# penn-graphics-research/claymore

Measured on AMD Instinct MI355X. Metric: particles*steps/sec, higher is better.
Workload: dtype f32

## Files before the change

claymore_amd/csrc/claymore_hip.hip:

```cpp
#include <hip/hip_runtime.h>

#include <algorithm>
#include <cmath>
#include <cstdio>
#include <cstdlib>
#include <chrono>
#include <cstring>
#include <string>
#include <vector>

#include "../../include/claymore_amd.h"
#include "mpm_kernels.hpp"
#include "mpm_readout.hpp"

using namespace mpm;
#define MPM_STR_(x) #x
#define MPM_STR(x) MPM_STR_(x)

namespace {
constexpr int kHaloWords	 = 128;
constexpr int kStatusBlock = ST_WORDS + kHaloWords + kMaxVelSlots * kMaxVelStride;

struct Partition {
	int* table = nullptr;
// ... 99 lines not shown
		}
	}
};

#define HIP_TRY(expr)                                                                                            \
	do {                                                                                                         \
		hipError_t e_ = (expr);                                                                                  \
		if(e_ != hipSuccess) {                                                                                   \
			ctx->err = std::string(#expr) + " -> " + hipGetErrorString(e_) + " (" + __FILE__ + ":" + std::to_string(__LINE__) + ")"; \
			return MPM_ERR_DEVICE;                                                                               \
		}                                                                                                        \
	} while(0)

static float host_maxvel(const mpm_ctx* ctx) {
	float m = 0.f;
	for(int i = 0; i < kMaxVelSlots; ++i) m = std::max(m, ctx->h_maxvel[i * kMaxVelStride]);
	return m;
}

#ifndef MPM_PAIR_BUILD
#define MPM_PAIR_BUILD 0xF
#endif
#ifndef MPM_PAIR_DEFAULT
#define MPM_PAIR_DEFAULT 0xF
#endif
static int pair_mask() {
	static const int mask = [] {
		const char* e = std::getenv("MPM_G2P2G_PAIRS");
		return (e && *e ? (int) std::strtol(e, nullptr, 0) : MPM_PAIR_DEFAULT) & MPM_PAIR_BUILD;
	}();
	return mask;
}

static int launch_prepare(mpm_ctx* ctx, int cur, int prev, bool list_is_out, int binoff_sel, const int* pbc_ptr, int nblocks_est, bool sort, bool publish);

static int fail(mpm_ctx* ctx, int code, const std::string& msg) {
	ctx->err = msg;
	return code;
}

static inline void phase_call(mpm_ctx* ctx) {
	if(ctx) ctx->group_summed = false;
}

template<typename T>
static hipError_t dalloc(T** p, size_t n) {
	return hipMalloc((void**) p, sizeof(T) * (n ? n : 1));
}

template<typename T>
struct DevScratch {
	T* p = nullptr;
	DevScratch() = default;
	DevScratch(const DevScratch&) = delete;
	DevScratch& operator=(const DevScratch&) = delete;
	~DevScratch() {
		if(p) hipFree(p);
	}
	hipError_t alloc(size_t n) { return dalloc(&p, n); }
};

template<typename T>
static hipError_t regrow(T** p, size_t old_n, size_t new_n, hipStream_t s) {
	T* q		 = nullptr;
	hipError_t e = hipMalloc((void**) &q, sizeof(T) * new_n);
	if(e != hipSuccess) return e;
	if((e = hipMemsetAsync(q, 0, sizeof(T) * new_n, s)) != hipSuccess || (*p && old_n && (e = hipMemcpyAsync(q, *p, sizeof(T) * old_n, hipMemcpyDeviceToDevice, s)) != hipSuccess)
// ... 246 lines not shown
	HIP_TRY(hipMemsetAsync(ctx->d_status, 0, sizeof(int) * kStatusBlock, s));
	for(int i = 0; i < 2; ++i) {
		HIP_TRY(dalloc(&ctx->part[i].table, table));
		HIP_TRY(dalloc(&ctx->part[i].count, 1));
		HIP_TRY(hipMemsetAsync(ctx->part[i].table, 0xff, sizeof(int) * table, s));
		HIP_TRY(hipMemsetAsync(ctx->part[i].count, 0, sizeof(int), s));
	}
	size_t total_particles = 0;
	for(auto& m: ctx->models) total_particles += m.n;
	size_t prov = std::min(table, total_particles + 1);
	if(ctx->cfg.max_blocks > 0) prov = std::min<size_t>(table, (size_t) ctx->cfg.max_blocks);
	Partition& P = ctx->part[n];
	HIP_TRY(dalloc(&P.keys, 3 * prov));
	g.cap = (int) prov;
	for(auto& m: ctx->models)
		if(m.n) activate_blocks_kernel<<<cdiv(m.n, 256), 256, 0, s>>>(g, m.n, m.d_xyz, P.table, P.keys, P.count, ctx->d_status);
	int pbc = 0;
	HIP_TRY(hipMemcpyAsync(&pbc, P.count, sizeof(int), hipMemcpyDeviceToHost, s));
	HIP_TRY(hipStreamSynchronize(s));
	if(pbc > g.cap) return fail(ctx, MPM_ERR_CAPACITY, "Too much active blocks: " + std::to_string(pbc));
	ctx->pbc = pbc;
	if(ctx->cfg.max_blocks <= 0 && (size_t) pbc * 27 > prov) {
		int* keys		  = nullptr;
		const size_t need = std::min(table, (size_t) pbc * 27 + 1);
		HIP_TRY(dalloc(&keys, 3 * need));
		HIP_TRY(hipMemcpyAsync(keys, P.keys, sizeof(int) * 3 * (size_t) pbc, hipMemcpyDeviceToDevice, s));
		HIP_TRY(hipStreamSynchronize(s));
		HIP_TRY(hipFree(P.keys));
		P.keys = keys;
		prov   = need;
		g.cap  = (int) prov;
	}
	HIP_TRY(hipMemcpyAsync(&ctx->d_status[ST_CNT_P], P.count, sizeof(int), hipMemcpyDeviceToDevice, s));
	register_blocks_kernel<0, 1><<<std::max(1u, std::min(4096u, cdiv((size_t) pbc * 8, 256))), 256, 0, s>>>(g, &ctx->d_status[ST_CNT_P], nullptr, &ctx->d_status[ST_CNT_N], &ctx->d_status[ST_PBC], P.table, P.keys, ctx->d_status);
	register_blocks_kernel<-1, 1><<<std::max(1u, std::min(8192u, cdiv((size_t) pbc * 32, 256))), 256, 0, s>>>(g, &ctx->d_status[ST_CNT_P], &ctx->d_status[ST_CNT_N], &ctx->d_status[ST_CNT_E], &ctx->d_status[ST_NBC], P.table, P.keys, ctx->d_status);
	{
		int rc0 = read_status(ctx);
		if(rc0) return rc0;
		rc0 = check_status(ctx);
		if(rc0) return rc0;
		const int ebc0 = ctx->h_status[ST_CNT_P] + ctx->h_status[ST_CNT_N] + ctx->h_status[ST_CNT_E];
		ctx->h_status[ST_EBC] = ebc0;
		ctx->pbc_prev		  = pbc;
		HIP_TRY(hipMemcpyAsync(&ctx->d_status[ST_EBC], &ctx->h_status[ST_EBC], sizeof(int), hipMemcpyHostToDevice, s));
		HIP_TRY(hipMemcpyAsync(&ctx->d_status[ST_PBCPREV], &ctx->pbc_prev, sizeof(int), hipMemcpyHostToDevice, s));
		HIP_TRY(hipMemcpyAsync(P.count, &ctx->h_status[ST_EBC], sizeof(int), hipMemcpyHostToDevice, s));
		HIP_TRY(hipStreamSynchronize(s));
	}
	ctx->nbc = ctx->h_status[ST_NBC];
	ctx->ebc = ctx->h_status[ST_EBC];
	size_t cap = ctx->cfg.max_blocks > 0 ? (size_t) ctx->cfg.max_blocks : std::min(table, (size_t) ctx->ebc * 3 / 2 + 4096);
	if(cap < (size_t) ctx->ebc) return fail(ctx, MPM_ERR_CAPACITY, "Too much exterior blocks: " + std::to_string(ctx->ebc) + " (max_blocks " + std::to_string(cap) + ")");
	{
		int* keys = nullptr;
		HIP_TRY(dalloc(&keys, 3 * cap));
		HIP_TRY(hipMemcpyAsync(keys, P.keys, sizeof(int) * 3 * (size_t) ctx->ebc, hipMemcpyDeviceToDevice, s));
		HIP_TRY(hipStreamSynchronize(s));
		HIP_TRY(hipFree(P.keys));
		P.keys = keys;
		HIP_TRY(dalloc(&ctx->part[r].keys, 3 * cap));
	}
	g.cap = (int) cap;
	for(int i = 0; i < 2; ++i) {
		HIP_TRY(dalloc(&ctx->grid[i], cap * 256));
	}
	for(size_t mi = 0; mi < ctx->models.size(); ++mi) {
		Model& m  = ctx->models[mi];
		m.bin_cap = m.n / kBin + cap + 1;
// ... 197 lines not shown
		for(auto& m: ctx->models) launch_g2p2g_model(ctx, m, nullptr, &ctx->d_status[ST_PBC], ctx->pbc, dt, next_dt, s);
	HIP_TRY(hipEventRecord(e1, s));
	return MPM_OK;
}

int mpm_g2p2g(mpm_ctx* ctx, float dt, float next_dt) {
	phase_call(ctx);
	if(!ctx || !ctx->ready) return MPM_ERR_NOT_READY;
	HIP_TRY(hipSetDevice(ctx->device));
	int rc = launch_g2p2g(ctx, dt, next_dt, ctx->ev.g2p2g_start, ctx->ev.g2p2g_end);
	if(rc) return rc;
	HIP_TRY(hipGetLastError());
	HIP_TRY(hipStreamSynchronize(ctx->s_compute));
	HIP_TRY(hipEventElapsedTime(&ctx->last_g2p2g_ms, ctx->ev.g2p2g_start, ctx->ev.g2p2g_end));
	ctx->timers.g2p2g_ms = ctx->last_g2p2g_ms;
	return MPM_OK;
}

static int launch_prepare(mpm_ctx* ctx, int cur, int prev, bool list_is_out, int binoff_sel, const int* pbc_ptr, int nblocks_est, bool sort, bool publish) {
	if(nblocks_est <= 0 && !publish) return MPM_OK;
	PrepareModels pm {};
	pm.n = (int) ctx->models.size();
	for(int mi = 0; mi < pm.n; ++mi) {
		Model& m		  = ctx->models[mi];
		pm.list[mi]		  = m.list[list_is_out ? (m.list_in ^ 1) : m.list_in];
		pm.size[mi]		  = m.size;
		pm.row_of[mi]	  = m.row_of;
		pm.binoff_src[mi] = m.binoff[binoff_sel];
		pm.blockinfo[mi]  = m.blockinfo;
		pm.keep[mi]		  = sort && list_is_out ? m.keep : nullptr;
		pm.pairinfo[mi]	  = m.pair ? m.pairinfo[0] : nullptr;
		pm.pairhand[mi]	  = m.pairinfo[1];
	}
	const int nwg = std::max(1, std::min(ctx->g.cap, nblocks_est + nblocks_est / 16 + 64));
	int* pub	  = publish ? ctx->d_status : nullptr;
	if(sort)
		prepare_blocks_kernel<true><<<nwg, 64, 0, ctx->s_compute>>>(ctx->g, pm, pbc_ptr, ctx->part[cur].table, ctx->part[cur].keys, ctx->part[prev].table, pub, ctx->part[cur].count);
	else
		prepare_blocks_kernel<false><<<nwg, 64, 0, ctx->s_compute>>>(ctx->g, pm, pbc_ptr, ctx->part[cur].table, ctx->part[cur].keys, ctx->part[prev].table, pub, ctx->part[cur].count);
	return MPM_OK;
}

static int launch_rebuild_prepare(mpm_ctx* ctx) {
	const int r = ctx->rollid, n = r ^ 1;
	const int ebc_est = std::min(ctx->g.cap, ctx->ebc + ctx->ebc / 16 + 1024);
	return launch_prepare(ctx, n, r, true, n, &ctx->d_status[ST_CNT_P], ebc_est, true, true);
}
static int launch_rebuild(mpm_ctx* ctx, float fuse_dt = 0.f, bool without_prepare = false) {
	if(fuse_dt == 0.f) fuse_dt = ctx->fuse_dt_once;
	ctx->fuse_dt_once = 0.f;
	hipStream_t s = ctx->s_compute;
	GridCfg& g	  = ctx->g;
	const int r = ctx->rollid, n = r ^ 1;
	Partition& Pn = ctx->part[n];
	Partition& Pr = ctx->part[r];
	const bool fused = fuse_dt > 0.f;
	ctx->grid_momentum = !fused;
	int rc			 = launch_clear(ctx, kClearRebuild | (fused ? kClearMaxVel : 0));
	if(rc) return rc;
	RebuildModels rm {};
	rm.n = (int) ctx->models.size();
	for(int mi = 0; mi < rm.n; ++mi) {
		Model& m		 = ctx->models[mi];
		rm.out_count[mi] = m.out_count;
		rm.size[mi]		 = m.size;
		rm.row_of[mi]	 = m.row_of;
		rm.binoff[mi]	 = m.binoff[r];
		rm.bin_cap[mi]	 = (long long) m.bin_cap;
	}
	int* st			  = ctx->d_status;
	const int ebc_est = std::min(g.cap, ctx->ebc + ctx->ebc / 16 + 1024);
	compact_blocks_kernel<<<std::max(1u, cdiv(ebc_est, 1024)), 1024, 0, s>>>(g, rm, Pr.keys, Pn.keys, Pn.table, st);
	const unsigned rg8 = std::max(1u, std::min(4096u, cdiv((size_t) ebc_est * 8, 256))), rg32 = std::max(1u, std::min(8192u, cdiv((size_t) ebc_est * 32, 256)));
	register_blocks_kernel<0, 1><<<rg8, 256, 0, s>>>(g, &st[ST_CNT_P], nullptr, &st[ST_CNT_N], &st[ST_PBC], Pn.table, Pn.keys, st);
	if(fused) {
		if(ctx->has_collision)
			carry_grid_kernel<true, true><<<2048, 256, 0, s>>>(g, st, Pn.keys, Pr.table, ctx->grid[1], ctx->grid[0], fuse_dt, ctx->d_maxvel, collision_tick(ctx, fuse_dt));
		else
			carry_grid_kernel<true><<<2048, 256, 0, s>>>(g, st, Pn.keys, Pr.table, ctx->grid[1], ctx->grid[0], fuse_dt, ctx->d_maxvel, NoCollision {});
		ctx->grid_preupdated = true;
		ctx->preupdate_dt	 = fuse_dt;
	} else
		carry_grid_kernel<false><<<2048, 256, 0, s>>>(g, st, Pn.keys, Pr.table, ctx->grid[1], ctx->grid[0], 0.f, nullptr, NoCollision {});
	register_blocks_kernel<-1, 1><<<rg32, 256, 0, s>>>(g, &st[ST_CNT_P], &st[ST_CNT_N], &st[ST_CNT_E], &st[ST_NBC], Pn.table, Pn.keys, st);
	if(without_prepare) return MPM_OK;
	return launch_prepare(ctx, n, r, true, n, &st[ST_CNT_P], ebc_est, true, true);
}

static int grow_capacity(mpm_ctx* ctx) {
	if(!ctx->cfg.grow) return MPM_OK;
	hipStream_t s	   = ctx->s_compute;
	const size_t table = (size_t) ctx->g.G * ctx->g.G * ctx->g.G;
	const size_t cap   = (size_t) ctx->g.cap;
	if((size_t) ctx->ebc * 4 > cap * 3 && cap < table) {
		const size_t ncap = std::min(table, cap * 3 / 2 + 1);
		HIP_TRY(hipDeviceSynchronize());
		for(int i = 0; i < 2; ++i) {
			HIP_TRY(regrow(&ctx->part[i].keys, 3 * cap, 3 * ncap, s));
			HIP_TRY(regrow(&ctx->grid[i], cap * 256, ncap * 256, s));
		}
		for(auto& m: ctx->models) {
			for(int i = 0; i < 2; ++i) {
				HIP_TRY(regrow(&m.binoff[i], cap + 1, ncap + 1, s));
				HIP_TRY(regrow(&m.list[i], cap * (size_t) ctx->g.ppb, ncap * (size_t) ctx->g.ppb, s));
			}
			HIP_TRY(regrow(&m.size, cap + 1, ncap + 1, s));
			HIP_TRY(regrow(&m.row_of, cap + 1, ncap + 1, s));
			HIP_TRY(regrow(&m.out_count, cap + 1, ncap + 1, s));
			HIP_TRY(regrow(&m.keep, cap + 1, ncap + 1, s));
			HIP_TRY(regrow(&m.blockinfo, cap * (size_t) kInfoRow, ncap * (size_t) kInfoRow, s));
			if(m.pair)
				for(int i = 0; i < 2; ++i) HIP_TRY(regrow(&m.pairinfo[i], (cap + 1) * (size_t) kPairChunks, (ncap + 1) * (size_t) kPairChunks, s));
		}
		if(ctx->d_overlap) {
			HIP_TRY(regrow(&ctx->d_overlap, cap + 1, ncap + 1, s));
			HIP_TRY(regrow(&ctx->d_halo_list, cap + 1, ncap + 1, s));
			HIP_TRY(regrow(&ctx->d_inner_list, cap + 1, ncap + 1, s));
// ... 524 lines not shown
```

claymore_amd/csrc/mpm_g2p2g.hpp:

```cpp
#pragma once
#include "mpm_device_math.hpp"

namespace mpm {

#if !(defined(MPM_EXPERIMENT) && defined(MPM_G2P2G_WAVES_FLUID))
#define MPM_G2P2G_WAVES_FLUID 4
#endif
#if !(defined(MPM_EXPERIMENT) && defined(MPM_G2P2G_WAVES))
#define MPM_G2P2G_WAVES 3
#endif

constexpr int kP2GStrideX = 36, kP2GStrideY = 6, kP2GNodes = 216;
constexpr int kP2GArena2 = 228;
constexpr int kG2PStrideX = 6, kG2PStrideY = 1, kG2PStrideZ = 36, kG2PNodes = 216;

struct ModelView {
	const float* bins_src;
	float* bins_dst;
	const int* binoff_src;
	const int* binoff_dst;
	const int* list_in;
	int* list_out;
	const int* size;
	const int* row_of;
// ... 364 lines not shown
	float am;
	StressScale ss;
	float jdiv, jvisc;
	float refl_lim;
};

MPM_DEV int code_key(int c) {
	return ((c >> 4) & 15) * 36 + (c & 15) * 6 + (c >> 8);
}
MPM_DEV bool code_edge(int c) {
	const int x = c & 15, y = (c >> 4) & 15, z = c >> 8;
	return (x == 0) | (x == 5) | (y == 0) | (y == 5) | (z == 0) | (z == 5);
}
MPM_DEV int code_off(int c) {
	return ((c & 15) - 1) * kP2GStrideX + (((c >> 4) & 15) - 1) * kP2GStrideY + ((c >> 8) - 1);
}

template<int MAT>
__global__ __launch_bounds__(kG2P2GThreads, MAT == 0 ? MPM_G2P2G_WAVES_FLUID : MPM_G2P2G_WAVES) void g2p2g_kernel(GridCfg cfg, ModelView mv, const int* __restrict__ cur_keys, const float* __restrict__ grid, float* __restrict__ next_grid, const int* __restrict__ block_list, const int* __restrict__ only_flag, const int* __restrict__ nblocks_ptr, int nblocks, float dt, float new_dt, StepConst sk, int* __restrict__ status) {
	constexpr int NCH = MatTraits<MAT>::nch;
	constexpr int REC = MatTraits<MAT>::rec;
	__shared__ float4 g2p[kG2PNodes];
	__shared__ float4 p2g[kP2GArena2 + kP2GNodes];
	__shared__ unsigned char s_owner[2 * 216];
	constexpr bool kQueue = MAT != 0 && kSerialQueue > 0;
	__shared__ float4 s_queue[kQueue ? 4 * kSerialQueue : 1];
#if defined(MPM_EXPERIMENT) && defined(MPM_LDS_PAD)
	__shared__ float s_pad[MPM_LDS_PAD / 4];
	if(size_t(grid) == 1) s_pad[threadIdx.x] = 0.f;
#endif

	const int lane0 = threadIdx.x;
	const int total = nblocks_ptr ? min(*nblocks_ptr, cfg.cap) : nblocks;
	const int xcd = (int) (blockIdx.x & 7u), nq = nblocks_ptr ? (int) (gridDim.x >> 3) : 0x40000000;
	const int share = (total >> 3) + (xcd < (total & 7) ? 1 : 0);
	const int first = xcd * (total >> 3) + min(xcd, total & 7);
	for(int q = (int) (blockIdx.x >> 3); q < share; q += nq) {
	int lane = lane0;
	__asm__ volatile("" : "+v"(lane));
	const int bid = first + q;
	const int b	  = block_list ? block_list[bid] : bid;
	const int size		 = mv.size[b];
	const int row		 = mv.row_of[b];
	const int binoff_dst = mv.binoff_dst[b];
	const int flag = only_flag ? only_flag[b] : 1;
	if(size == 0 || flag == 0) continue;
	const int* list		= mv.list_in + (size_t) row * cfg.ppb;
	const float mass	= mv.mc.mass;
	const int key_shift = cfg.pid_bits;
	const int tag_shift = cfg.pid_bits + kKeyBits;
	const int info = mv.blockinfo[(size_t) b * kInfoRow + lane];
	int cnt_cur	   = slice_records_at(size, 0);
	int cnt_next   = 64 < size ? slice_records_at(size, 64) : 1;
	int rec_cur	   = list[min(lane, cnt_cur - 1)];
	int rec_next   = list[(64 < size ? 64 : 0) + min(lane, cnt_next - 1)];
	for(int i = lane; i < kP2GArena2 + kP2GNodes; i += 64) p2g[i] = make_float4(0.f, 0.f, 0.f, 0.f);
	__syncthreads();
	float4 gv[8];
#pragma unroll
	for(int lb = 0; lb < 8; ++lb) {
		const int nb	= __shfl(info, 54 + lb);
		const float* gb = grid + (size_t) (nb < 0 ? 0 : nb) * 256;
		gv[lb].x		= gb[64 + lane];
		gv[lb].y		= gb[128 + lane];
		gv[lb].z		= gb[192 + lane];
		if(nb < 0) gv[lb].x = gv[lb].y = gv[lb].z = 0.f;
		gv[lb].w = gv[lb].z;
	}
	constexpr int ROW = NCH - REC;
// ... 321 lines not shown
```

claymore_amd/csrc/mpm_g2p2g_pair.hpp:

```cpp
#pragma once
#include "mpm_g2p2g.hpp"

namespace mpm {

#if !(defined(MPM_EXPERIMENT) && defined(MPM_PAIR_WAVES))
#define MPM_PAIR_WAVES 3
#endif
#if !(defined(MPM_EXPERIMENT) && defined(MPM_PAIR_WAVES_FLUID))
#define MPM_PAIR_WAVES_FLUID 4
#endif
#if !(defined(MPM_EXPERIMENT) && defined(MPM_PAIR_DUAL))
#define MPM_PAIR_DUAL 0
#endif
#if !(defined(MPM_EXPERIMENT) && defined(MPM_PAIR_LATE_FETCH_FLUID))
#define MPM_PAIR_LATE_FETCH_FLUID 1
#endif
#if !(defined(MPM_EXPERIMENT) && defined(MPM_PAIR_LATE_FETCH_NACC))
#define MPM_PAIR_LATE_FETCH_NACC 1
#endif
#if !(defined(MPM_EXPERIMENT) && defined(MPM_PAIR_LATE_FETCH))
#define MPM_PAIR_LATE_FETCH 0
#endif
#if !(defined(MPM_EXPERIMENT) && defined(MPM_PAIR_SHARED_GATHER))
#define MPM_PAIR_SHARED_GATHER 0x0
// ... 244 lines not shown
		const int i = o / 9, j = (o / 3) % 3, k = o % 3;
		node0[i * kP2GStrideX + j * kP2GStrideY + k] = make_float4(a01.x, a01.y, a23.x, a23.y);
		__asm__ volatile("" ::: "memory");
		if(o + 1 < 27) {
			const int i1 = (o + 1) / 9, j1 = ((o + 1) / 3) % 3, k1 = (o + 1) % 3;
			acc			 = node0[i1 * kP2GStrideX + j1 * kP2GStrideY + k1];
		}
	}
	template<int SITE>
	MPM_DEV void at() {
		static_assert(SITE >= 0 && SITE < NSITES, "site out of range");
		if(win) {
#pragma unroll
			for(int o = SITE * 27 / NSITES; o < (SITE + 1) * 27 / NSITES; ++o) step(o);
		}
	}
#endif
};

template<int MAT>
__global__ __launch_bounds__(kG2P2GThreads, MAT == 0 ? MPM_PAIR_WAVES_FLUID : MPM_PAIR_WAVES) void g2p2g_pair_kernel(GridCfg cfg, ModelView mv, const int* __restrict__ cur_keys, const float* __restrict__ grid, float* __restrict__ next_grid, const int* __restrict__ block_list, const int* __restrict__ only_flag, const int* __restrict__ nblocks_ptr, int nblocks, float dt, float new_dt, StepConst sk, int* __restrict__ status) {
	constexpr int NCH = MatTraits<MAT>::nch;
	constexpr int REC = MatTraits<MAT>::rec;
	constexpr bool kSharedGather = ((MPM_PAIR_SHARED_GATHER >> MAT) & 1) != 0;
	constexpr int kLateFetch	 = MAT == 0 ? MPM_PAIR_LATE_FETCH_FLUID : (MAT == 3 ? MPM_PAIR_LATE_FETCH_NACC : MPM_PAIR_LATE_FETCH);
	__shared__ float4 g2p[kG2PNodes];
	__shared__ float4 p2g[kP2GArena2 + kP2GNodes];
	__shared__ unsigned char s_owner[2 * 216];
	constexpr bool kQueue = MAT != 0 && kSerialQueue > 0;
	__shared__ float4 s_queue[kQueue ? 4 * kSerialQueue : 1];

	const int lane0 = threadIdx.x;
	const int total = nblocks_ptr ? min(*nblocks_ptr, cfg.cap) : nblocks;
	const int xcd = (int) (blockIdx.x & 7u), nq = nblocks_ptr ? (int) (gridDim.x >> 3) : 0x40000000;
	const int share = (total >> 3) + (xcd < (total & 7) ? 1 : 0);
	const int first = xcd * (total >> 3) + min(xcd, total & 7);
	for(int q = (int) (blockIdx.x >> 3); q < share; q += nq) {
	int lane = lane0;
	__asm__ volatile("" : "+v"(lane));
	const int bid = first + q;
	const int b	  = block_list ? block_list[bid] : bid;
	const int size		 = mv.size[b];
	const int row		 = mv.row_of[b];
	const int binoff_dst = mv.binoff_dst[b];
	const int flag		 = only_flag ? only_flag[b] : 1;
	if(size == 0 || flag == 0) continue;
	const int* list		= mv.list_in + (size_t) row * cfg.ppb;
	const float mass	= mv.mc.mass;
	const int key_shift = cfg.pid_bits;
	const int tag_shift = cfg.pid_bits + kKeyBits;
	const int info		= mv.blockinfo[(size_t) b * kInfoRow + lane];
	int chunk_nrec;
	{
		const int nch = pair_chunks(size), cl = lane & (kPairChunks - 1);
		chunk_nrec	  = cl < nch ? (cl + 1 < nch ? 512 : size - 512 * cl) : 0;
	}
	const int pinfo		= (mv.pairinfo_in[(size_t) b * kPairChunks + (lane & (kPairChunks - 1))] & 0xffff) | (chunk_nrec << 16);
	int d_slice = 0;
	auto form_slices = [&](int first) {
		int before = 0;
		d_slice = 0;
#pragma unroll 1
		for(int c = 0; c < kPairChunks; ++c) {
			const int pe = __builtin_amdgcn_readlane(pinfo, c);
			if((pe >> 16) == 0) break;
			const PairChunk pc = pair_chunk(pe >> 16, pe & 0xffff);
			const int t		   = first + lane - before;
			if(t >= 0 && t < pc.S) {
				int pos, ca, cb;
// ... 404 lines not shown
```

claymore_amd/csrc/mpm_kernels.hpp:

```cpp
#pragma once
#include <hip/hip_runtime.h>
#include <type_traits>

#include "mpm_device_math.hpp"
#include "mpm_collision.hpp"

namespace mpm {

constexpr int kBin		  = 64;
constexpr int kG2P2GThreads = 64;
constexpr int kMaxModels  = 8;
constexpr int kSortKeys		= 216;
constexpr int kKeyBits		= 8;
constexpr int kStay		  = 13;

enum {
	ST_PBC = 0, ST_NBC = 1, ST_EBC = 2, ST_OVERFLOW = 3, ST_LOST = 4, ST_ARENA = 5, ST_DROPPED = 6, ST_NONFINITE = 7, ST_BINS0 = 8, ST_PART0 = 16,
	 ST_CNT_P = 29, ST_CNT_N = 30, ST_CNT_E = 31, ST_BINSPREV = 32, ST_PBCPREV = 40, ST_WORDS = 64
};

struct GridCfg {
	int G;
	int gbits;
	int ppb;
	int pid_bits;
	int boundary;
	int cap;
	float dx, dx_inv, d_inv, gravity;
};

__device__ __forceinline__ bool key_ok(const GridCfg& c, int x, int y, int z) {
	return ((unsigned) x < (unsigned) c.G) & ((unsigned) y < (unsigned) c.G) & ((unsigned) z < (unsigned) c.G);
}
__device__ __forceinline__ size_t key_index(const GridCfg& c, int x, int y, int z) {
	return ((size_t) x << (2 * c.gbits)) | ((size_t) y << c.gbits) | (size_t) z;
}
__device__ __forceinline__ int table_query(const GridCfg& c, const int* __restrict__ table, int x, int y, int z) {
	return key_ok(c, x, y, z) ? table[key_index(c, x, y, z)] : -1;
}
__device__ __forceinline__ void table_insert(const GridCfg& c, int* table, int* keys, int* count, int x, int y, int z, int* status) {
	if(!key_ok(c, x, y, z)) return;
	const size_t i = key_index(c, x, y, z);
	if(table[i] != -1) return;
	if(atomicCAS(&table[i], -1, -2) == -1) {
		const int idx = atomicAdd(count, 1);
		if(idx < c.cap) {
			table[i]		 = idx;
			keys[3 * idx]	 = x;
			keys[3 * idx + 1] = y;
			keys[3 * idx + 2] = z;
		} else {
			table[i] = -1;
			atomicOr(&status[ST_OVERFLOW], 1);
		}
	}
}

__device__ __forceinline__ int wave_append(int* counter, bool pred) {
	const unsigned long long m = __ballot(pred);
	if(m == 0ull) return -1;
	const int lane	 = threadIdx.x & 63;
	const int leader = __ffsll((long long) m) - 1;
	int base		 = 0;
	if(lane == leader) base = atomicAdd(counter, __popcll(m));
	base = __shfl(base, leader);
	return pred ? base + __popcll(m & ((1ull << lane) - 1ull)) : -1;
}


__device__ __forceinline__ int wave_scan_incl(int v) {
	v += __builtin_amdgcn_update_dpp(0, v, 0x111, 0xf, 0xf, false);
// ... 226 lines not shown
	if(i < n) out[i] = make_float4(sd[i], gx[i], gy[i], gz[i]);
}

__device__ __forceinline__ void dir_components(int dir, int& dx, int& dy, int& dz) {
	dz = (dir % 3) - 1;
	dy = ((dir / 3) % 3) - 1;
	dx = (dir / 9) - 1;
}

constexpr int kInfoRow = 64;
struct PrepareModels {
	int n;
	int* list[kMaxModels];
	const int* size[kMaxModels];
	const int* row_of[kMaxModels];
	const int* binoff_src[kMaxModels];
	int* blockinfo[kMaxModels];
	const int* keep[kMaxModels];
	int* pairinfo[kMaxModels];
	const int* pairhand[kMaxModels];
};
template<bool SORT>
__global__ __launch_bounds__(64) void prepare_blocks_kernel(GridCfg cfg, PrepareModels pm, const int* __restrict__ pbc_ptr, const int* __restrict__ cur_table, const int* __restrict__ cur_keys, const int* __restrict__ prev_table, int* __restrict__ publish, int* __restrict__ part_count) {
	constexpr int kPrepChunk = kListChunk;
	__shared__ int s_sorted[kPairChunkMax];
	__shared__ int s_cnt[256];
	__shared__ int s_cur[256];
	const int lane = threadIdx.x;
	if(publish && blockIdx.x == 0 && lane == 0) {
		const int ebc	 = publish[ST_CNT_P] + publish[ST_CNT_N] + publish[ST_CNT_E];
		publish[ST_EBC] = ebc;
		*part_count		 = ebc;
	}
	const int pbc = min(*pbc_ptr, cfg.cap);
	for(int b = blockIdx.x; b < pbc; b += gridDim.x) {
	const int kx = cur_keys[3 * b], ky = cur_keys[3 * b + 1], kz = cur_keys[3 * b + 2];
	int size0 = 0, row0 = 0, keep0 = -2, hand0 = 0;
	if constexpr(SORT) {
		if(pm.n > 0) {
			size0 = pm.size[0][b];
			row0  = pm.row_of[0][b];
			if(pm.keep[0]) keep0 = pm.keep[0][row0];
			if(pm.pairinfo[0]) hand0 = pm.pairhand[0][(size_t) row0 * kPairChunks + (lane & (kPairChunks - 1))];
		}
	}
	int srcno = -1, other = -1;
	if(lane < 27) {
		int ox, oy, oz;
		dir_components(lane, ox, oy, oz);
		srcno = table_query(cfg, prev_table, kx + ox, ky + oy, kz + oz);
	} else if(lane < 54) {
		int ox, oy, oz;
		dir_components(lane - 27, ox, oy, oz);
		other = table_query(cfg, cur_table, kx - ox, ky - oy, kz - oz);
	} else if(lane < 62) {
		const int lb = lane - 54;
		other		 = table_query(cfg, cur_table, kx + ((lb >> 2) & 1), ky + ((lb >> 1) & 1), kz + (lb & 1));
	}
	const int key_shift		= cfg.pid_bits;
	const int tag_shift		= cfg.pid_bits + kKeyBits;
	const unsigned rec_mask = (1u << (tag_shift + 5)) - 1u;
	for(int m = 0; m < pm.n; ++m) {
		int info = other;
		if constexpr(SORT) {
		const int size = __builtin_amdgcn_readfirstlane(m == 0 ? size0 : pm.size[m][b]);
		const int row  = __builtin_amdgcn_readfirstlane(m == 0 ? row0 : pm.row_of[m][b]);
		int* list	   = pm.list[m] + (size_t) row * cfg.ppb;
		const int tail	= size & (kPrepChunk - 1);
// ... 203 lines not shown
enum { kClearP2G = 1, kClearRebuild = 2, kClearMaxVel = 4 };
struct ClearArgs {
	int flags;
	int nmodels;
	int* out_count[kMaxModels];
	int* keep[kMaxModels];
	float* p2g_grid;
	int* status;
	unsigned* max_vel_bits;
	int* old_table;
	const int* old_keys;
	const int* old_count;
};
__global__ __launch_bounds__(256) void substep_clear_kernel(GridCfg cfg, ClearArgs a) {
	const int tid = blockIdx.x * 256 + threadIdx.x, nthreads = gridDim.x * 256;
	if(a.flags & kClearP2G) {
		const int nbc = min(a.status[ST_NBC], cfg.cap), ebc = min(a.status[ST_EBC], cfg.cap);
		float4* g	  = reinterpret_cast<float4*>(a.p2g_grid);
		for(int i = tid; i < nbc * 64; i += nthreads) g[i] = make_float4(0.f, 0.f, 0.f, 0.f);
		for(int m = 0; m < a.nmodels; ++m)
			for(int i = tid; i <= ebc; i += nthreads) a.out_count[m][i] = 0, a.keep[m][i] = -1;
	}
	if(a.flags & kClearRebuild) {
		const int n = min(*a.old_count, cfg.cap);
		for(int i = tid; i < n; i += nthreads) a.old_table[key_index(cfg, a.old_keys[3 * i], a.old_keys[3 * i + 1], a.old_keys[3 * i + 2])] = -1;
		if(blockIdx.x == gridDim.x - 1) {
			if(threadIdx.x < kMaxModels) {
				a.status[ST_BINSPREV + threadIdx.x] = a.status[ST_BINS0 + threadIdx.x];
				a.status[ST_BINS0 + threadIdx.x]	= 0;
				a.status[ST_PART0 + threadIdx.x]	= 0;
			}
			if(threadIdx.x >= 8 && threadIdx.x < 11) a.status[ST_CNT_P + threadIdx.x - 8] = 0;
			if(threadIdx.x == 11) a.status[ST_PBCPREV] = a.status[ST_PBC];
			if(threadIdx.x >= 64 && threadIdx.x < 64 + kMaxVelSlots) {
				unsigned* slot = a.max_vel_bits + (threadIdx.x - 64) * kMaxVelStride;
				if(*slot >= 0x7f800000u) a.status[ST_NONFINITE] = 1;
				if(a.flags & kClearMaxVel) *slot = 0u;
			}
		}
	}
}

__global__ __launch_bounds__(1024) void compact_blocks_kernel(GridCfg cfg, RebuildModels rm, const int* __restrict__ old_keys, int* __restrict__ new_keys, int* __restrict__ new_table, int* __restrict__ status) {
	__shared__ int s_part[kMaxModels];
	const int ebc = min(status[ST_EBC], cfg.cap);
	for(int b0 = blockIdx.x * blockDim.x; b0 < ebc; b0 += gridDim.x * blockDim.x) {
		const int b = b0 + threadIdx.x;
		int c[kMaxModels];
		bool any = false;
		for(int m = 0; m < rm.n; ++m) {
			c[m] = b < ebc ? rm.out_count[m][b] : 0;
			if(c[m] > cfg.ppb) {
				atomicAdd(&status[ST_DROPPED], c[m] - cfg.ppb);
				c[m] = cfg.ppb;
			}
			any |= c[m] > 0;
		}
		__syncthreads();
		if(threadIdx.x < kMaxModels) s_part[threadIdx.x] = 0;
		__syncthreads();
		for(int m = 0; m < rm.n; ++m) {
			int t = c[m];
#pragma unroll
			for(int off = 32; off > 0; off >>= 1) t += __shfl_xor(t, off);
			if((threadIdx.x & 63) == 0 && t) atomicAdd(&s_part[m], t);
		}
		__syncthreads();
		if((int) threadIdx.x < rm.n && s_part[threadIdx.x]) atomicAdd(&status[ST_PART0 + threadIdx.x], s_part[threadIdx.x]);
		const int nb = block_append(&status[ST_CNT_P], any ? 1 : 0);
		int kx = 0, ky = 0, kz = 0;
		if(any) {
			kx = old_keys[3 * b], ky = old_keys[3 * b + 1], kz = old_keys[3 * b + 2];
			new_keys[3 * nb]					  = kx;
			new_keys[3 * nb + 1]				  = ky;
			new_keys[3 * nb + 2]				  = kz;
			new_table[key_index(cfg, kx, ky, kz)] = nb;
		}
		for(int m = 0; m < rm.n; ++m) {
			const int nbins = any ? (c[m] + kBin - 1) / kBin : 0;
			const int first = block_append(&status[ST_BINS0 + m], nbins);
			if(any) {
				const bool fits = (long long) first + nbins <= rm.bin_cap[m];
				if(!fits) atomicOr(&status[ST_OVERFLOW], 4);
				rm.size[m][nb]	 = fits ? c[m] : 0;
				rm.row_of[m][nb] = b;
				rm.binoff[m][nb] = (nbins && fits) ? first : 0;
			}
		}
	}
}

template<int LO, int HI>
__global__ __launch_bounds__(256) void register_blocks_kernel(GridCfg cfg, const int* __restrict__ pbc_ptr, const int* __restrict__ base2_ptr, int* counter, int* publish, int* table, int* keys, int* status) {
	constexpr int W	   = HI - LO + 1;
	constexpr int NOFF = W * W * W;
	constexpr int LPB  = NOFF <= 8 ? 8 : 32;
	const int pbc	   = min(*pbc_ptr, cfg.cap);
	const int base	   = *pbc_ptr + (base2_ptr ? *base2_ptr : 0);
	if(publish && blockIdx.x == 0 && threadIdx.x == 0) *publish = base;
	const long long total = (long long) pbc * LPB;
	const long long bound = (total + blockDim.x - 1) / blockDim.x * blockDim.x;
	for(long long t = (long long) blockIdx.x * blockDim.x + threadIdx.x; t < bound; t += (long long) gridDim.x * blockDim.x) {
		const int b = (int) (t / LPB), o = (int) (t % LPB);
		bool claim	= false;
		int x = 0, y = 0, z = 0;
		size_t i = 0;
		if(t < total && o < NOFF) {
			x = keys[3 * b] + LO + o / (W * W);
			y = keys[3 * b + 1] + LO + (o / W) % W;
			z = keys[3 * b + 2] + LO + o % W;
			if(key_ok(cfg, x, y, z)) {
				i = key_index(cfg, x, y, z);
				if(table[i] == -1) claim = atomicCAS(&table[i], -1, -2) == -1;
			}
		}
		const int idx = base + block_append(counter, claim ? 1 : 0);
		if(claim) {
			if(idx < cfg.cap) {
				table[i]		  = idx;
				keys[3 * idx]	  = x;
				keys[3 * idx + 1] = y;
				keys[3 * idx + 2] = z;
			} else {
				table[i] = -1;
				atomicOr(&status[ST_OVERFLOW], 1);
			}
		}
	}
}

template<bool UPDATE, bool COLLIDE = false>
__global__ __launch_bounds__(256) void carry_grid_kernel(GridCfg cfg, const int* __restrict__ status, const int* __restrict__ new_keys, const int* __restrict__ old_table, const float* __restrict__ p2g_grid, float* __restrict__ grid, float dt, unsigned* __restrict__ max_vel_bits, std::conditional_t<COLLIDE, CollisionArgs, NoCollision> col) {
	static_assert(UPDATE || !COLLIDE, "the collision object belongs to the grid update");
	const int nbc	  = min(status[ST_CNT_P] + status[ST_CNT_N], cfg.cap);
	const int old_nbc = min(status[ST_NBC], cfg.cap);
	const int lane = threadIdx.x & 63;
	float vel_sqr  = 0.f;
	for(int nb = blockIdx.x * 4 + (threadIdx.x >> 6); nb < nbc; nb += gridDim.x * 4) {
		const int kx = new_keys[3 * nb], ky = new_keys[3 * nb + 1], kz = new_keys[3 * nb + 2];
		const int old = table_query(cfg, old_table, kx, ky, kz);
		float4 v	  = {0.f, 0.f, 0.f, 0.f};
		if(old >= 0 && old < old_nbc) {
			const float* s = p2g_grid + (size_t) old * 256;
			v			   = {s[lane], s[64 + lane], s[128 + lane], s[192 + lane]};
		}
		if constexpr(COLLIDE) {
			if(v.x > 0.0f) vel_sqr = fmaxf(vel_sqr, grid_cell_collision(cfg, col, kx, ky, kz, lane, dt, v));
		} else if constexpr(UPDATE) {
			if(v.x > 0.0f) {
				const bool wx = kx < cfg.boundary || kx >= cfg.G - cfg.boundary;
				const bool wy = ky < cfg.boundary || ky >= cfg.G - cfg.boundary;
				const bool wz = kz < cfg.boundary || kz >= cfg.G - cfg.boundary;
				const float mass_inv = 1.f / v.x;
				const float v0		 = wx ? 0.0f : v.y * mass_inv;
				const float v1		 = (wy ? 0.0f : v.z * mass_inv) + cfg.gravity * dt;
				const float v2		 = wz ? 0.0f : v.w * mass_inv;
				v.y					 = v0;
				v.z					 = v1;
				v.w					 = v2;
				float q				 = v0 * v0 + v1 * v1 + v2 * v2;
				if(q != q) q = __builtin_inff();
				vel_sqr = fmaxf(vel_sqr, q);
			}
		}
		float* d	  = grid + (size_t) nb * 256;
		d[lane]		  = v.x;
		d[64 + lane]  = v.y;
		d[128 + lane] = v.z;
		d[192 + lane] = v.w;
	}
	if constexpr(UPDATE) {
#pragma unroll
		for(int off = 32; off > 0; off >>= 1) vel_sqr = fmaxf(vel_sqr, __shfl_xor(vel_sqr, off));
		if(lane == 0 && vel_sqr > 0.f) {
			const unsigned bits = __float_as_uint(vel_sqr);
			unsigned* slot		= max_vel_bits + (blockIdx.x & (kMaxVelSlots - 1)) * kMaxVelStride;
			if(bits > __hip_atomic_load(slot, __ATOMIC_RELAXED, __HIP_MEMORY_SCOPE_AGENT)) atomicMax(slot, bits);
		}
	}
}

__device__ __forceinline__ void particle_block_key(const GridCfg& cfg, const float* xyz, size_t i, int& bx, int& by, int& bz, int& cellx, int& celly, int& cellz) {
	cellx = node_index(xyz[3 * i], cfg.dx_inv) - 2;
	celly = node_index(xyz[3 * i + 1], cfg.dx_inv) - 2;
	cellz = node_index(xyz[3 * i + 2], cfg.dx_inv) - 2;
	bx	  = cellx / 4;
	by	  = celly / 4;
	bz	  = cellz / 4;
}
__global__ void activate_blocks_kernel(GridCfg cfg, size_t n, const float* __restrict__ xyz, int* table, int* keys, int* count, int* status) {
	const size_t i = (size_t) blockIdx.x * blockDim.x + threadIdx.x;
	if(i >= n) return;
	int bx, by, bz, cx, cy, cz;
	particle_block_key(cfg, xyz, i, bx, by, bz, cx, cy, cz);
	table_insert(cfg, table, keys, count, bx, by, bz, status);
}
__global__ void bucket_particles_kernel(GridCfg cfg, size_t n, const float* __restrict__ xyz, const int* __restrict__ table, int* counts, int* ids, int* status) {
	const size_t i = (size_t) blockIdx.x * blockDim.x + threadIdx.x;
	if(i >= n) return;
	int bx, by, bz, cx, cy, cz;
	particle_block_key(cfg, xyz, i, bx, by, bz, cx, cy, cz);
	const int bno = table_query(cfg, table, bx, by, bz);
	if(bno < 0) {
		atomicAdd(&status[ST_LOST], 1);
		return;
	}
	const int slot = atomicAdd(&counts[bno], 1);
	if(slot >= cfg.ppb) {
		atomicOr(&status[ST_OVERFLOW], 2);
		return;
	}
	ids[(size_t) bno * cfg.ppb + slot] = (int) i;
// ... 133 lines not shown
```

Baseline: 34.39 billion.

## Fuse grid carry with exterior block registration and partition work per XCD

In the fused rebuild path, the carry_grid kernel and the exterior register_blocks kernel are merged into one launch. Workgroups split by role: every third group per XCD registers blocks and the rest carry grid data. Registration, prepare and carry loops now hand each XCD a contiguous range of blocks, and launch sizes are rounded up to a multiple of 8. Carry reads the previous NBC from a new snapshot slot because registration now runs concurrently and overwrites ST_NBC. The aim is to save a kernel launch and serialization and to improve L2 locality per XCD, at the cost of a fixed role ratio that may load-balance poorly.

```diff
diff --git a/claymore_amd/csrc/claymore_hip.hip b/claymore_amd/csrc/claymore_hip.hip
--- a/claymore_amd/csrc/claymore_hip.hip
+++ b/claymore_amd/csrc/claymore_hip.hip
@@ -155,7 +155,18 @@
 	return mask;
 }
 
+static bool carry_split() {
+	static const bool split = [] {
+		const char* e = std::getenv("MPM_CARRY_SPLIT");
+		return e && e[0] == '1';
+	}();
+	return split;
+}
+
 static int launch_prepare(mpm_ctx* ctx, int cur, int prev, bool list_is_out, int binoff_sel, const int* pbc_ptr, int nblocks_est, bool sort, bool publish);
+static inline unsigned xcd_launch(size_t nwg) {
+	return (unsigned) ((std::max<size_t>(nwg, 1) + 7) & ~(size_t) 7);
+}
 
 static int fail(mpm_ctx* ctx, int code, const std::string& msg) {
 	ctx->err = msg;
@@ -468,8 +479,8 @@
 		g.cap  = (int) prov;
 	}
 	HIP_TRY(hipMemcpyAsync(&ctx->d_status[ST_CNT_P], P.count, sizeof(int), hipMemcpyDeviceToDevice, s));
-	register_blocks_kernel<0, 1><<<std::max(1u, std::min(4096u, cdiv((size_t) pbc * 8, 256))), 256, 0, s>>>(g, &ctx->d_status[ST_CNT_P], nullptr, &ctx->d_status[ST_CNT_N], &ctx->d_status[ST_PBC], P.table, P.keys, ctx->d_status);
-	register_blocks_kernel<-1, 1><<<std::max(1u, std::min(8192u, cdiv((size_t) pbc * 32, 256))), 256, 0, s>>>(g, &ctx->d_status[ST_CNT_P], &ctx->d_status[ST_CNT_N], &ctx->d_status[ST_CNT_E], &ctx->d_status[ST_NBC], P.table, P.keys, ctx->d_status);
+	register_blocks_kernel<0, 1><<<xcd_launch(std::min(4096u, cdiv((size_t) pbc * 8, 256))), 256, 0, s>>>(g, &ctx->d_status[ST_CNT_P], nullptr, &ctx->d_status[ST_CNT_N], &ctx->d_status[ST_PBC], P.table, P.keys, ctx->d_status);
+	register_blocks_kernel<-1, 1><<<xcd_launch(std::min(8192u, cdiv((size_t) pbc * 32, 256))), 256, 0, s>>>(g, &ctx->d_status[ST_CNT_P], &ctx->d_status[ST_CNT_N], &ctx->d_status[ST_CNT_E], &ctx->d_status[ST_NBC], P.table, P.keys, ctx->d_status);
 	{
 		int rc0 = read_status(ctx);
 		if(rc0) return rc0;
@@ -733,7 +744,7 @@
 		pm.pairinfo[mi]	  = m.pair ? m.pairinfo[0] : nullptr;
 		pm.pairhand[mi]	  = m.pairinfo[1];
 	}
-	const int nwg = std::max(1, std::min(ctx->g.cap, nblocks_est + nblocks_est / 16 + 64));
+	const unsigned nwg = xcd_launch((size_t) std::max(1, std::min(ctx->g.cap, nblocks_est + nblocks_est / 16 + 64)));
 	int* pub	  = publish ? ctx->d_status : nullptr;
 	if(sort)
 		prepare_blocks_kernel<true><<<nwg, 64, 0, ctx->s_compute>>>(ctx->g, pm, pbc_ptr, ctx->part[cur].table, ctx->part[cur].keys, ctx->part[prev].table, pub, ctx->part[cur].count);
@@ -772,18 +783,26 @@
 	int* st			  = ctx->d_status;
 	const int ebc_est = std::min(g.cap, ctx->ebc + ctx->ebc / 16 + 1024);
 	compact_blocks_kernel<<<std::max(1u, cdiv(ebc_est, 1024)), 1024, 0, s>>>(g, rm, Pr.keys, Pn.keys, Pn.table, st);
-	const unsigned rg8 = std::max(1u, std::min(4096u, cdiv((size_t) ebc_est * 8, 256))), rg32 = std::max(1u, std::min(8192u, cdiv((size_t) ebc_est * 32, 256)));
+	const unsigned rg8 = xcd_launch(std::min(4096u, cdiv((size_t) ebc_est * 8, 256))), rg32 = xcd_launch(std::min(8192u, cdiv((size_t) ebc_est * 32, 256)));
 	register_blocks_kernel<0, 1><<<rg8, 256, 0, s>>>(g, &st[ST_CNT_P], nullptr, &st[ST_CNT_N], &st[ST_PBC], Pn.table, Pn.keys, st);
 	if(fused) {
-		if(ctx->has_collision)
-			carry_grid_kernel<true, true><<<2048, 256, 0, s>>>(g, st, Pn.keys, Pr.table, ctx->grid[1], ctx->grid[0], fuse_dt, ctx->d_maxvel, collision_tick(ctx, fuse_dt));
+		const bool split = carry_split();
+		if(ctx->has_collision) {
+			if(split)
+				carry_grid_kernel<true, true><<<2048, 256, 0, s>>>(g, st, Pn.keys, Pr.table, ctx->grid[1], ctx->grid[0], fuse_dt, ctx->d_maxvel, collision_tick(ctx, fuse_dt));
+			else
+				carry_register_kernel<true, true><<<kCarryRegisterGrid, 256, 0, s>>>(g, st, Pn.keys, Pn.table, Pr.table, ctx->grid[1], ctx->grid[0], fuse_dt, ctx->d_maxvel, collision_tick(ctx, fuse_dt));
+		} else if(split)
+			carry_grid_kernel<true><<<2048, 256, 0, s>>>(g, st, Pn.keys, Pr.table, ctx->grid[1], ctx->grid[0], fuse_dt, ctx->d_maxvel, NoCollision {});
 		else
-			carry_grid_kernel<true><<<2048, 256, 0, s>>>(g, st, Pn.keys, Pr.table, ctx->grid[1], ctx->grid[0], fuse_dt, ctx->d_maxvel, NoCollision {});
+			carry_register_kernel<true><<<kCarryRegisterGrid, 256, 0, s>>>(g, st, Pn.keys, Pn.table, Pr.table, ctx->grid[1], ctx->grid[0], fuse_dt, ctx->d_maxvel, NoCollision {});
+		if(split) register_blocks_kernel<-1, 1><<<rg32, 256, 0, s>>>(g, &st[ST_CNT_P], &st[ST_CNT_N], &st[ST_CNT_E], &st[ST_NBC], Pn.table, Pn.keys, st);
 		ctx->grid_preupdated = true;
 		ctx->preupdate_dt	 = fuse_dt;
-	} else
+	} else {
 		carry_grid_kernel<false><<<2048, 256, 0, s>>>(g, st, Pn.keys, Pr.table, ctx->grid[1], ctx->grid[0], 0.f, nullptr, NoCollision {});
-	register_blocks_kernel<-1, 1><<<rg32, 256, 0, s>>>(g, &st[ST_CNT_P], &st[ST_CNT_N], &st[ST_CNT_E], &st[ST_NBC], Pn.table, Pn.keys, st);
+		register_blocks_kernel<-1, 1><<<rg32, 256, 0, s>>>(g, &st[ST_CNT_P], &st[ST_CNT_N], &st[ST_CNT_E], &st[ST_NBC], Pn.table, Pn.keys, st);
+	}
 	if(without_prepare) return MPM_OK;
 	return launch_prepare(ctx, n, r, true, n, &st[ST_CNT_P], ebc_est, true, true);
 }
diff --git a/claymore_amd/csrc/mpm_g2p2g.hpp b/claymore_amd/csrc/mpm_g2p2g.hpp
--- a/claymore_amd/csrc/mpm_g2p2g.hpp
+++ b/claymore_amd/csrc/mpm_g2p2g.hpp
@@ -420,9 +420,8 @@
 
 	const int lane0 = threadIdx.x;
 	const int total = nblocks_ptr ? min(*nblocks_ptr, cfg.cap) : nblocks;
-	const int xcd = (int) (blockIdx.x & 7u), nq = nblocks_ptr ? (int) (gridDim.x >> 3) : 0x40000000;
-	const int share = (total >> 3) + (xcd < (total & 7) ? 1 : 0);
-	const int first = xcd * (total >> 3) + min(xcd, total & 7);
+	const XcdShare xs = xcd_share(total, nblocks_ptr != nullptr);
+	const int nq = xs.nq, share = xs.share, first = xs.first;
 	for(int q = (int) (blockIdx.x >> 3); q < share; q += nq) {
 	int lane = lane0;
 	__asm__ volatile("" : "+v"(lane));
diff --git a/claymore_amd/csrc/mpm_g2p2g_pair.hpp b/claymore_amd/csrc/mpm_g2p2g_pair.hpp
--- a/claymore_amd/csrc/mpm_g2p2g_pair.hpp
+++ b/claymore_amd/csrc/mpm_g2p2g_pair.hpp
@@ -300,9 +300,8 @@
 
 	const int lane0 = threadIdx.x;
 	const int total = nblocks_ptr ? min(*nblocks_ptr, cfg.cap) : nblocks;
-	const int xcd = (int) (blockIdx.x & 7u), nq = nblocks_ptr ? (int) (gridDim.x >> 3) : 0x40000000;
-	const int share = (total >> 3) + (xcd < (total & 7) ? 1 : 0);
-	const int first = xcd * (total >> 3) + min(xcd, total & 7);
+	const XcdShare xs = xcd_share(total, nblocks_ptr != nullptr);
+	const int nq = xs.nq, share = xs.share, first = xs.first;
 	for(int q = (int) (blockIdx.x >> 3); q < share; q += nq) {
 	int lane = lane0;
 	__asm__ volatile("" : "+v"(lane));
diff --git a/claymore_amd/csrc/mpm_kernels.hpp b/claymore_amd/csrc/mpm_kernels.hpp
--- a/claymore_amd/csrc/mpm_kernels.hpp
+++ b/claymore_amd/csrc/mpm_kernels.hpp
@@ -16,7 +16,7 @@
 
 enum {
 	ST_PBC = 0, ST_NBC = 1, ST_EBC = 2, ST_OVERFLOW = 3, ST_LOST = 4, ST_ARENA = 5, ST_DROPPED = 6, ST_NONFINITE = 7, ST_BINS0 = 8, ST_PART0 = 16,
-	 ST_CNT_P = 29, ST_CNT_N = 30, ST_CNT_E = 31, ST_BINSPREV = 32, ST_PBCPREV = 40, ST_WORDS = 64
+	 ST_CNT_P = 29, ST_CNT_N = 30, ST_CNT_E = 31, ST_BINSPREV = 32, ST_PBCPREV = 40, ST_NBCPREV = 41, ST_WORDS = 64
 };
 
 struct GridCfg {
@@ -37,6 +37,17 @@
 }
 __device__ __forceinline__ int table_query(const GridCfg& c, const int* __restrict__ table, int x, int y, int z) {
 	return key_ok(c, x, y, z) ? table[key_index(c, x, y, z)] : -1;
+}
+struct XcdShare {
+	int first, share, nq;
+};
+__device__ __forceinline__ XcdShare xcd_share(int total, bool walk = true) {
+	const int xcd = (int) (blockIdx.x & 7u);
+	XcdShare xs;
+	xs.nq	 = walk ? (int) (gridDim.x >> 3) : 0x40000000;
+	xs.share = (total >> 3) + (xcd < (total & 7) ? 1 : 0);
+	xs.first = xcd * (total >> 3) + min(xcd, total & 7);
+	return xs;
 }
 __device__ __forceinline__ void table_insert(const GridCfg& c, int* table, int* keys, int* count, int x, int y, int z, int* status) {
 	if(!key_ok(c, x, y, z)) return;
@@ -329,8 +340,9 @@
 		publish[ST_EBC] = ebc;
 		*part_count		 = ebc;
 	}
-	const int pbc = min(*pbc_ptr, cfg.cap);
-	for(int b = blockIdx.x; b < pbc; b += gridDim.x) {
+	const XcdShare xs = xcd_share(min(*pbc_ptr, cfg.cap));
+	for(int q = (int) (blockIdx.x >> 3); q < xs.share; q += xs.nq) {
+	const int b	 = xs.first + q;
 	const int kx = cur_keys[3 * b], ky = cur_keys[3 * b + 1], kz = cur_keys[3 * b + 2];
 	int size0 = 0, row0 = 0, keep0 = -2, hand0 = 0;
 	if constexpr(SORT) {
@@ -600,6 +612,7 @@
 			}
 			if(threadIdx.x >= 8 && threadIdx.x < 11) a.status[ST_CNT_P + threadIdx.x - 8] = 0;
 			if(threadIdx.x == 11) a.status[ST_PBCPREV] = a.status[ST_PBC];
+			if(threadIdx.x == 12) a.status[ST_NBCPREV] = a.status[ST_NBC];
 			if(threadIdx.x >= 64 && threadIdx.x < 64 + kMaxVelSlots) {
 				unsigned* slot = a.max_vel_bits + (threadIdx.x - 64) * kMaxVelStride;
 				if(*slot >= 0x7f800000u) a.status[ST_NONFINITE] = 1;
@@ -659,16 +672,17 @@
 }
 
 template<int LO, int HI>
-__global__ __launch_bounds__(256) void register_blocks_kernel(GridCfg cfg, const int* __restrict__ pbc_ptr, const int* __restrict__ base2_ptr, int* counter, int* publish, int* table, int* keys, int* status) {
+MPM_DEV void register_blocks_body(const GridCfg& cfg, int q0, int nq, const int* __restrict__ pbc_ptr, const int* __restrict__ base2_ptr, int* counter, int* publish, int* table, int* keys, int* status) {
 	constexpr int W	   = HI - LO + 1;
 	constexpr int NOFF = W * W * W;
 	constexpr int LPB  = NOFF <= 8 ? 8 : 32;
 	const int pbc	   = min(*pbc_ptr, cfg.cap);
 	const int base	   = *pbc_ptr + (base2_ptr ? *base2_ptr : 0);
-	if(publish && blockIdx.x == 0 && threadIdx.x == 0) *publish = base;
+	if(publish && q0 == 0 && (blockIdx.x & 7u) == 0 && threadIdx.x == 0) *publish = base;
 	const long long total = (long long) pbc * LPB;
-	const long long bound = (total + blockDim.x - 1) / blockDim.x * blockDim.x;
-	for(long long t = (long long) blockIdx.x * blockDim.x + threadIdx.x; t < bound; t += (long long) gridDim.x * blockDim.x) {
+	const XcdShare xs	  = xcd_share((int) ((total + blockDim.x - 1) / blockDim.x));
+	for(int q = q0; q < xs.share; q += nq) {
+		const long long t = (long long) (xs.first + q) * blockDim.x + threadIdx.x;
 		const int b = (int) (t / LPB), o = (int) (t % LPB);
 		bool claim	= false;
 		int x = 0, y = 0, z = 0;
@@ -696,15 +710,22 @@
 		}
 	}
 }
-
-template<bool UPDATE, bool COLLIDE = false>
-__global__ __launch_bounds__(256) void carry_grid_kernel(GridCfg cfg, const int* __restrict__ status, const int* __restrict__ new_keys, const int* __restrict__ old_table, const float* __restrict__ p2g_grid, float* __restrict__ grid, float dt, unsigned* __restrict__ max_vel_bits, std::conditional_t<COLLIDE, CollisionArgs, NoCollision> col) {
+template<int LO, int HI>
+__global__ __launch_bounds__(256) void register_blocks_kernel(GridCfg cfg, const int* __restrict__ pbc_ptr, const int* __restrict__ base2_ptr, int* counter, int* publish, int* table, int* keys, int* status) {
+	register_blocks_body<LO, HI>(cfg, (int) (blockIdx.x >> 3), (int) (gridDim.x >> 3), pbc_ptr, base2_ptr, counter, publish, table, keys, status);
+}
+
+template<bool UPDATE, bool COLLIDE>
+MPM_DEV void carry_grid_body(const GridCfg& cfg, int q0, int nq, const int* __restrict__ status, const int* __restrict__ new_keys, const int* __restrict__ old_table, const float* __restrict__ p2g_grid, float* __restrict__ grid, float dt, unsigned* __restrict__ max_vel_bits, const std::conditional_t<COLLIDE, CollisionArgs, NoCollision>& col) {
 	static_assert(UPDATE || !COLLIDE, "the collision object belongs to the grid update");
 	const int nbc	  = min(status[ST_CNT_P] + status[ST_CNT_N], cfg.cap);
-	const int old_nbc = min(status[ST_NBC], cfg.cap);
+	const int old_nbc = min(status[ST_NBCPREV], cfg.cap);
 	const int lane = threadIdx.x & 63;
 	float vel_sqr  = 0.f;
-	for(int nb = blockIdx.x * 4 + (threadIdx.x >> 6); nb < nbc; nb += gridDim.x * 4) {
+	const XcdShare xs = xcd_share((nbc + 3) >> 2);
+	for(int q = q0; q < xs.share; q += nq) {
+		const int nb = (xs.first + q) * 4 + (threadIdx.x >> 6);
+		if(nb >= nbc) break;
 		const int kx = new_keys[3 * nb], ky = new_keys[3 * nb + 1], kz = new_keys[3 * nb + 2];
 		const int old = table_query(cfg, old_table, kx, ky, kz);
 		float4 v	  = {0.f, 0.f, 0.f, 0.f};
@@ -726,9 +747,9 @@
 				v.y					 = v0;
 				v.z					 = v1;
 				v.w					 = v2;
-				float q				 = v0 * v0 + v1 * v1 + v2 * v2;
-				if(q != q) q = __builtin_inff();
-				vel_sqr = fmaxf(vel_sqr, q);
+				float q2			 = v0 * v0 + v1 * v1 + v2 * v2;
+				if(q2 != q2) q2 = __builtin_inff();
+				vel_sqr = fmaxf(vel_sqr, q2);
 			}
 		}
 		float* d	  = grid + (size_t) nb * 256;
@@ -746,6 +767,22 @@
 			if(bits > __hip_atomic_load(slot, __ATOMIC_RELAXED, __HIP_MEMORY_SCOPE_AGENT)) atomicMax(slot, bits);
 		}
 	}
+}
+template<bool UPDATE, bool COLLIDE = false>
+__global__ __launch_bounds__(256) void carry_grid_kernel(GridCfg cfg, const int* __restrict__ status, const int* __restrict__ new_keys, const int* __restrict__ old_table, const float* __restrict__ p2g_grid, float* __restrict__ grid, float dt, unsigned* __restrict__ max_vel_bits, std::conditional_t<COLLIDE, CollisionArgs, NoCollision> col) {
+	carry_grid_body<UPDATE, COLLIDE>(cfg, (int) (blockIdx.x >> 3), (int) (gridDim.x >> 3), status, new_keys, old_table, p2g_grid, grid, dt, max_vel_bits, col);
+}
+
+constexpr int kRoleStride		 = 3;
+constexpr int kCarryRegisterGrid = 2048;
+template<bool UPDATE, bool COLLIDE = false>
+__global__ __launch_bounds__(256) void carry_register_kernel(GridCfg cfg, int* __restrict__ status, int* __restrict__ new_keys, int* __restrict__ new_table, const int* __restrict__ old_table, const float* __restrict__ p2g_grid, float* __restrict__ grid, float dt, unsigned* __restrict__ max_vel_bits, std::conditional_t<COLLIDE, CollisionArgs, NoCollision> col) {
+	const int g = (int) (blockIdx.x >> 3), ng = (int) (gridDim.x >> 3);
+	const int nreg = (ng + kRoleStride - 1) / kRoleStride;
+	if(g % kRoleStride == 0)
+		register_blocks_body<-1, 1>(cfg, g / kRoleStride, nreg, &status[ST_CNT_P], &status[ST_CNT_N], &status[ST_CNT_E], &status[ST_NBC], new_table, new_keys, status);
+	else
+		carry_grid_body<UPDATE, COLLIDE>(cfg, g - g / kRoleStride - 1, ng - nreg, status, new_keys, old_table, p2g_grid, grid, dt, max_vel_bits, col);
 }
 
 __device__ __forceinline__ void particle_block_key(const GridCfg& cfg, const float* xyz, size_t i, int& bx, int& by, int& bz, int& cellx, int& celly, int& cellz) {
```

Measured after the change: 34.69 billion, median of 6. No clear change (+0.9%).
